# nygenome/Lancet2

Measured on AMD Instinct MI355X. Metric: microassembly windows/sec (whole node), higher is better.
Workload: dtype u8/i32 (f64 statistics)

## Files before the change

### lancet2_amd/csrc/assemble.hip

```cpp
#include <algorithm>
#include <cstdio>
#include <cstdlib>
#include <utility>
#include <vector>

#include "graph_ws.h"

namespace ma {

int run_build_pass(ma_ctx* ctx, const DBatch& b, GraphWs& ws, u32* counters_dev, int tc_log2_alloc);
int run_count_inst(ma_ctx* ctx, const DBatch& b, const GraphWs& ws, int win0, int nwin, u32* maxima_dev);
int run_select_active(ma_ctx* ctx, const GraphWs& ws, int win0, int nwin, const u32* gate_approx, u32* win_k,
                      u32* active, u32* n_active_dev);
int run_clean_pass(ma_ctx* ctx, const DBatch& b, const GraphWs& ws, const ma_asm_out_t& out);

namespace {

__global__ void k_init_out(ma_asm_out_t o, u32* win_flags, int n, u32 MC, u32 MH) {
  int const i = blockIdx.x * blockDim.x + threadIdx.x;
  if (i >= n) return;
  o.win_status[i] = MA_W_NO_HAPLOTYPE;
  o.win_k[i] = 0;
  o.win_ncomp[i] = 0;
  win_flags[i] = 0;
// ... 312 lines not shown

int launch_assemble(ma_ctx* ctx, const DBatch& b, const ma_asm_out_t& out, const u32* gate_approx) {
  int const n = b.n_windows;
  if (n == 0) return MA_OK;
  ma_params_t const& P = ctx->prm;
  int const S = P.num_samples;

  size_t const nseq = static_cast<size_t>(b.n_reads) + n;
  Carver cm{nullptr};
  auto carve_misc = [&](Carver& c, GraphWs& ws, u32** win_flags, u32** active, u32** counters) {
    ws.seq_inst_base = c.take<u32>(nseq + 1);
    ws.win_ninst = c.take<u32>(n);
    ws.win_nread_inst = c.take<u32>(n);
    *win_flags = c.take<u32>(n);
    *active = c.take<u32>(n);
    *counters = c.take<u32>(16);
    ws.rd_flag = c.take<u8>(static_cast<size_t>(b.n_reads) + 16);
  };
  GraphWs ws{};
  bool const nested = ctx->spec_k != nullptr;
  ws.win_kfirst = ctx->spec_k;
  u32 *win_flags = nullptr, *active = nullptr, *counters = nullptr;
  carve_misc(cm, ws, &win_flags, &active, &counters);
  MA_HIP(ctx, ctx->ws_nodes.reserve(cm.off + 4096));
  Carver cm2{static_cast<char*>(ctx->ws_nodes.p)};
  carve_misc(cm2, ws, &win_flags, &active, &counters);
  ws.win_flags = win_flags;
  ws.num_samples = S;

  hipLaunchKernelGGL(k_init_out, dim3((n + 63) / 64), dim3(64), 0, ctx->stream, out, win_flags, n, static_cast<u32>(P.max_comps),
                     static_cast<u32>(P.max_haps));
// ... 128 lines not shown
    size_t budget = stage_budget(0.60, ctx->ws_build.cap, size_t(48) << 30, ctx->hbm_share);
    if (const char* e = getenv("MA_WS_GB")) budget = static_cast<size_t>(atoi(e)) << 30;
    int chunk = static_cast<int>(std::max<size_t>(1, std::min<size_t>(n, budget / per_window)));
    MA_HIP(ctx, ctx->ws_build.reserve(per_window * static_cast<size_t>(chunk)));
    if (getenv("MA_VERBOSE"))
      fprintf(stderr, "[microasm] assemble: %d windows, %.2f MB/window, budget %.1f GB -> chunks of %d (nc %u, tc_log2 %d)\n", n,
              per_window / 1048576.0, budget / 1073741824.0, chunk, ws.nc, ws.tc_log2);

    for (int win0 = 0; win0 < n; win0 += chunk) {
      int const nwin = std::min(chunk, n - win0);
      ws.tc_log2 = tc_log2_alloc;
      ws.mc_log2 = mc_log2_alloc;
      Carver cw{static_cast<char*>(ctx->ws_build.p)};
      carve_ws(cw, ws, static_cast<size_t>(nwin));
      int const rungs = (P.max_k - P.min_k) / P.k_step + 1;
      for (int kpass = 0; kpass <= rungs; ++kpass) {
        MA_TRY_RC(run_select_active(ctx, ws, win0, nwin, gate_approx, out.win_k, active, counters + 8));
        u32 host_cnt[2] = {0, 0};
        MA_HIP(ctx, hipMemcpyAsync(host_cnt, counters + 8, 8, hipMemcpyDeviceToHost, ctx->stream));
        MA_HIP(ctx, ma_stream_sync(ctx));
        ws.n_active = static_cast<int>(host_cnt[0]);
        ws.active = active;
        if (host_cnt[1] == 0) break;
        if (!nested && kpass >= 1 && ws.n_active > 0 && static_cast<u32>(ws.n_active) <= kSpecPending && P.max_k > P.min_k &&
            !getenv("MA_NO_SPEC")) {
          u32 still = 0;
          MA_TRY_RC(speculate_tail(ctx, b, out, gate_approx, active, static_cast<u32>(ws.n_active), win_flags, counters + 8, &still));
          continue;
        }
        if (ws.n_active > 0) {
          if (!nested) ctx->stats[3] += static_cast<unsigned long long>(ws.n_active);
          if (nested || P.min_k != P.max_k) MA_TRY_RC(run_count_inst(ctx, b, ws, win0, nwin, counters));
          ws.tc_log2 = tc_log2_alloc;
          ws.mc_log2 = mc_log2_alloc;
          MA_TRY_RC(run_build_pass(ctx, b, ws, counters + 12, tc_log2_alloc));
          if (ctx->collect) {
            unsigned long long* acc = nullptr;
            MA_TRY_RC(ma_dev_stats(ctx, &acc));
            hipLaunchKernelGGL(k_workload_stats, dim3(ws.n_active), dim3(256), 0, ctx->stream, ws, acc);
          }
          MA_TRY_RC(run_clean_pass(ctx, b, ws, out));
        }
      }
    }
  }
  return MA_OK;
}

}
```

### lancet2_amd/csrc/build.hip

```cpp
#include "graph_ws.h"

namespace ma {

constexpr int kBT = 256;
__constant__ u64 c_phred_bits[256] = {
#include "../../include/ma_phred_lut.inc"
};

struct SeqInfo {
  u64 off;
  u32 len;
  u32 nk;
};

__device__ __forceinline__ u32 seq_count(const DBatch& b, int w) {
  return 1u + (b.read_win_off[w + 1] - b.read_win_off[w]);
}

__device__ __forceinline__ SeqInfo seq_info(const DBatch& b, int w, u32 s, int k) {
  SeqInfo si;
  if (s == 0) {
    si.off = b.ref_off[w];
    si.len = b.ref_off[w + 1] - b.ref_off[w];
  } else {
// ... 965 lines not shown
  i32* c_hint = reinterpret_cast<i32*>(c_ib + cache_cap);
  bool const cached = cache_cap != 0 && ns <= cache_cap;
  SeqInfo const rsi = seq_info(b, w, 0, k);
  for (u32 i = threadIdx.x; i < cnt_words; i += kSupT) l_cnt[i] = 0;
  for (u32 i = threadIdx.x; i < (kSupT / 64u) << ws.dd_log2; i += kSupT) l_dd[i] = 0;
  for (u32 i = threadIdx.x; i < xs_cap; i += kSupT) {
    l_xkey[i] = 0;
    l_xgrp[i] = 0;
  }
  if (threadIdx.x == 0) {
    xs_flag = ns > 65535u ? 1u : 0u;
    any_big = 0;
    gen_count = 0;
    genq_n = 0;
    edgeq_n = 0;
  }
  if (cached) {
    for (u32 sx = 1 + threadIdx.x; sx < ns; sx += kSupT) {
      u32 const r = b.read_win_off[w] + sx - 1;
      SeqInfo const si = seq_info(b, w, sx, k);
      c_meta[sx] = (b.read_flags[r] & 7u) | (ws.rd_flag[r] ? 8u : 0u) | (static_cast<u32>(b.read_sample[r]) << 8) | (min(si.nk, 0xFFFFu) << 16);
      c_qn[sx] = b.read_qname_id[r];
      c_ib[sx] = ws.seq_inst_base[base_idx + sx];
      c_hint[sx] = b.read_hint ? b.read_hint[r] : 0;
    }
  }
  __syncthreads();
  bool const hints = b.read_hint != nullptr && rsi.len <= ws.max_ref_len + 8;
  if (hints) {
    for (u32 s_idx = 1 + threadIdx.x; s_idx < ns; s_idx += kSupT) {
      u32 const r = b.read_win_off[w] + s_idx - 1;
      if (!(b.read_flags[r] & MA_RF_PASS)) continue;
      u32 const key = ((b.read_qname_id[r] << 1) | ((b.read_flags[r] & MA_RF_CASE) ? 1u : 0u)) + 1u;
      u32 h = (key * 2654435761u) >> xs_shift;
      bool done = false;
      for (u32 probe = 0; probe < xs_cap && !done; ++probe) {
        u32 cur = l_xkey[h];
        if (cur == 0) {
          u32 const old = atomicCAS(&l_xkey[h], 0u, key);
          if (old == 0) {
            l_xsmp[h] = b.read_sample[r];
            done = true;
            break;
          }
          cur = old;
        }
        if (cur == key) done = true; else h = (h + 1) & (xs_cap - 1);
      }
      if (!done) xs_flag = 1;
    }
  }
  __syncthreads();
  if (hints) {
    for (u32 s_idx = 1 + threadIdx.x; s_idx < ns; s_idx += kSupT) {
      u32 const r = b.read_win_off[w] + s_idx - 1;
      if (!(b.read_flags[r] & MA_RF_PASS)) continue;
      bool const leader = !(s_idx > 1 && same_group(b, r, r - 1));
      u32 const key = ((b.read_qname_id[r] << 1) | ((b.read_flags[r] & MA_RF_CASE) ? 1u : 0u)) + 1u;
      u32 h = (key * 2654435761u) >> xs_shift;
      for (u32 probe = 0; probe < xs_cap; ++probe) {
        u32 const cur = l_xkey[h];
        if (cur == key) {
          if (l_xsmp[h] != b.read_sample[r]) xs_flag = 1;
          if (leader && atomicAdd(&l_xgrp[h], 1u) != 0) xs_flag = 1;
          break;
        }
        if (cur == 0) break;
        h = (h + 1) & (xs_cap - 1);
      }
    }
  }
  if (hints && ns > kSeqCap) {
    for (u32 s_idx = 1 + kMmRunMax + threadIdx.x; s_idx < ns; s_idx += kSupT) {
      u32 const r = b.read_win_off[w] + s_idx - 1;
      u32 j = 0;
      while (j < kMmRunMax && same_group(b, r - j, r - j - 1)) ++j;
      if (j == kMmRunMax) xs_flag = 1;
    }
  }
  __syncthreads();
  bool const all_generic = !hints || xs_flag != 0;
  bool const qmode = !all_generic && !ws.mm_force_hbm && ns <= kSeqCap && tbl_log2(ws) <= 20;
  u32* const genq = ws.slowq + static_cast<size_t>(a) * ws.inst_stride;
  u32 const dd_cap = 1u << ws.dd_log2;
  uint2* const edgeq = reinterpret_cast<uint2*>(ws.slow_rec + static_cast<size_t>(a) * ws.inst_stride);

  u32* const l_leaders = l_mask;
  if (threadIdx.x == 0) n_leaders = 0;
  __syncthreads();
  for (u32 s_idx = 1 + threadIdx.x; s_idx < ns; s_idx += kSupT) {
    u32 const r0 = b.read_win_off[w] + s_idx - 1;
    if (!(b.read_flags[r0] & MA_RF_PASS)) continue;
    if (s_idx > 1 && same_group(b, r0, r0 - 1)) continue;
    l_leaders[atomicAdd(&n_leaders, 1u)] = s_idx;
    if (qmode) {
      u32 tot = 0;
      for (u32 j = 0; s_idx + j < ns && (j == 0 || same_group(b, r0, r0 + j)); ++j) tot += seq_info(b, w, s_idx + j, k).nk;
      if (tot > dd_cap / 4u * 3u) any_big = 1;
    }
  }
  __syncthreads();
  bool const qdedup = qmode && ws.graph_fused && !any_big && ws.win_nslots[a] <= kGrSlots;
  IPROF_T0();
  u32 const wave = threadIdx.x >> 6, lane = threadIdx.x & 63u;
  u32* const dd = l_dd + (wave << ws.dd_log2);
  u32 wave_gen = 0;
  auto same_group_c = [&](u32 sa, u32 sb) {
    u32 const ma_ = c_meta[sa], mb = c_meta[sb];
    return (mb & MA_RF_PASS) && c_qn[sa] == c_qn[sb] && ((ma_ ^ mb) & MA_RF_CASE) == 0 && ((ma_ ^ mb) & 0xFF00u) == 0;
  };
  for (u32 gi = wave; gi < n_leaders; gi += kSupT / 64) {
    u32 const s_idx = l_leaders[gi];
    u32 const r0 = b.read_win_off[w] + s_idx - 1;
    u32 gsize = 1;
    if (cached) {
      while (s_idx + gsize < ns && same_group_c(s_idx, s_idx + gsize)) gsize++;
    } else {
      while (s_idx + gsize < ns && same_group(b, r0, r0 + gsize)) gsize++;
    }
    bool generic = all_generic || gsize > 2;
    for (u32 gm = 0; gm < gsize && !generic; ++gm) {
      if (cached) {
        u32 const mt = c_meta[s_idx + gm];
        if ((mt & 8u) || (mt >> 16) > 32u * kMaskWords) generic = true;
      } else {
        SeqInfo const si = seq_info(b, w, s_idx + gm, k);
        if (ws.rd_flag[r0 + gm] || si.nk > 32u * kMaskWords) generic = true;
      }
    }
    u32 pre00 = 0, pre01 = 0, pre10 = 0, pre11 = 0;
    bool have_pre = cached && gsize <= 2;
    for (u32 gm = 0; gm < gsize && have_pre; ++gm) {
      u32 const nkc = c_meta[s_idx + gm] >> 16;
      if (nkc == 0xFFFFu || nkc > 128u) have_pre = false;
    }
    if (have_pre) {
      u32 const nka = c_meta[s_idx] >> 16, iba = c_ib[s_idx];
      pre00 = lane < nka ? inst_slot[iba + lane] : 0u;
      pre01 = 64u + lane < nka ? inst_slot[iba + 64u + lane] : 0u;
      if (gsize == 2) {
        u32 const nkb = c_meta[s_idx + 1] >> 16, ibb = c_ib[s_idx + 1];
        pre10 = lane < nkb ? inst_slot[ibb + lane] : 0u;
        pre11 = 64u + lane < nkb ? inst_slot[ibb + 64u + lane] : 0u;
      }
    }
    i32 hint0 = 0;
    u32 nk0 = 0;
    unsigned long long m0[kMaskWords / 2];
#pragma unroll
    for (int x = 0; x < kMaskWords / 2; ++x) m0[x] = 0;
    for (u32 gm = 0; gm < gsize; ++gm) {
      u32 const sx = s_idx + gm;
      u32 const r = r0 + gm;
      SeqInfo si;
      u32 ibase, smp, role;
      i32 hint_r;
      if (cached && (c_meta[sx] >> 16) != 0xFFFFu) {
        u32 const mt = c_meta[sx];
        si.nk = mt >> 16;
// ... 4 lines not shown
      } else {
        si = seq_info(b, w, sx, k);
        ibase = ws.seq_inst_base[base_idx + sx];
        smp = b.read_sample[r];
        role = (b.read_flags[r] & MA_RF_CASE) ? 1u : 0u;
        hint_r = hints ? b.read_hint[r] : 0;
      }
      if (si.nk == 0) continue;
      if (smp >= static_cast<u32>(S)) smp = S - 1;
      if (gm == 0) {
        hint0 = hints ? hint_r : 0;
        nk0 = si.nk;
      }
      for (u32 ob = 0; ob < si.nk; ob += 64) {
        u32 const o = ob + lane;
        u32 const word = have_pre ? (gm == 0 ? (ob == 0 ? pre00 : pre01) : (ob == 0 ? pre10 : pre11))
                                  : (o < si.nk ? inst_slot[ibase + o] : 0u);
        {
          u32 const dn = __shfl_down(word, 1, 64);
          u32 first_next;
          if (have_pre) first_next = ob == 0 ? __shfl(gm == 0 ? pre01 : pre11, 0, 64) : 0u;
          else first_next = ob + 64 < si.nk ? inst_slot[ibase + ob + 64] : 0u;
          u32 const nextw = lane == 63 ? first_next : dn;
          bool const pair = o + 1 < si.nk && !((word & kInstFast) && (nextw & kInstFast) &&
                                               (nextw & kInstSlotMask) == (word & kInstSlotMask) + 1u);
          unsigned long long const em = __ballot(pair);
          if (em) {
            u32 eb = 0;
            if (lane == 0) eb = atomicAdd(&edgeq_n, static_cast<u32>(__popcll(em)));
            eb = __shfl(eb, 0, 64);
            if (pair) edgeq[eb + static_cast<u32>(__popcll(em & ((1ull << lane) - 1ull)))] = edge_pack(ibase + o, word, nextw);
          }
        }
        bool const ef = (word & kInstErrFree) != 0;
        bool const to_gen = ef && (generic || !(word & kInstFast));
        u32 const p = word & kInstSlotMask;
        unsigned long long const gmask = __ballot(to_gen);
        if (qdedup) {
          if (gmask) {
            u32 const nslot = to_gen ? ((word & kInstFast) ? ref_slot_g[p] : p) : 0u;
            bool won = false;
            if (to_gen) {
              u32 const tag = gi + 1u, mine = (nslot << 11) | tag;
              u32 h = (nslot * 2654435761u) >> (32u - ws.dd_log2);
              for (;;) {
                u32 cur = dd[h];
// ... 3 lines not shown
                    won = true;
                    break;
                  }
                  cur = old;
                  if ((cur & 0x7FFu) != tag) continue;
                }
                if (cur == mine) break;
                h = (h + 1u) & (dd_cap - 1u);
              }
            }
            unsigned long long const wm = __ballot(won);
            if (wm) {
              u32 qb = 0;
              if (lane == 0) qb = atomicAdd(&genq_n, static_cast<u32>(__popcll(wm)));
              qb = __shfl(qb, 0, 64);
              if (won) genq[qb + static_cast<u32>(__popcll(wm & ((1ull << lane) - 1ull)))] = (nslot << 4) | (smp << 1) | role;
            }
          }
        } else if (qmode) {
          if (gmask) {
            u32 qb = 0;
            if (lane == 0) qb = atomicAdd(&genq_n, static_cast<u32>(__popcll(gmask)));
            qb = __shfl(qb, 0, 64);
            if (to_gen) {
              u32 const nslot = (word & kInstFast) ? ref_slot_g[p] : p;
              genq[qb + static_cast<u32>(__popcll(gmask & ((1ull << lane) - 1ull)))] = ((nslot << 11) | (s_idx - 1u)) + 1u;
            }
          }
        } else if (to_gen) {
          inst_slot[ibase + o] = word | kInstGen;
        }
        wave_gen += static_cast<u32>(__popcll(gmask));
        bool const fast = ef && !to_gen;
        bool dup = false;
        if (gm == 1 && nk0 > 0 && fast) {
          i64 const o0 = static_cast<i64>(p) - hint0;
          if (o0 >= 0 && o0 < static_cast<i64>(nk0)) {
            unsigned long long wd = 0;
#pragma unroll
            for (int x = 0; x < kMaskWords / 2; ++x) wd = (o0 >> 6) == x ? m0[x] : wd;
            dup = (wd >> (o0 & 63)) & 1ull;
// ... 8 lines not shown
        if (fast && !dup) {
          u32 const i1 = p * CW + smp, i2 = p * CW + S + role;
          atomicAdd(&l_cnt[i1 >> 1], 1u << ((i1 & 1u) * 16u));
          atomicAdd(&l_cnt[i2 >> 1], 1u << ((i2 & 1u) * 16u));
        }
      }
    }
  }
  if (lane == 0 && wave_gen) atomicAdd(&gen_count, wave_gen);
  IPROF_SYNC(27);
  if (threadIdx.x == 0) {
    bool const lds_ok = !all_generic && !ws.mm_force_hbm && (ns > kSeqCap || gen_count <= 4u * kMmLdsMax) && tbl_log2(ws) <= 20;
    ws.n_edgeq[a] = edgeq_n;
    ws.n_genq[a] = (qmode || qdedup) ? genq_n : 0u;
    ws.mm_mode[a] = qdedup ? (gen_count | 0x20000000u) : qmode ? (gen_count | 0x40000000u) : (gen_count | (lds_ok ? 0u : 0x80000000u));
    atomic_max_lazy(max_gen, gen_count);
    ws.mm_log2[a] = 0;
    if (!qmode && !lds_ok && gen_count) {
      atomic_max_lazy(max_gen + 1, gen_count);
      u32 lg = 10;
      while (lg < 31u && (1ull << lg) < static_cast<u64>(gen_count) * 4u / 3u + 16u) ++lg;
      unsigned long long const bytes = ((12ull << lg) + 255ull) & ~255ull;
      unsigned long long const at = atomicAdd(ws.mm_pool_used, bytes);
      if (at + bytes <= ws.mm_pool_bytes) {
        ws.mm_off[a] = at;
        ws.mm_log2[a] = lg;
      } else {
        atomicOr(&ws.win_flags[w], 4u);
      }
    }
// ... 823 lines not shown
__host__ __device__ inline u32 graph_lds_bytes(u32 inst_stride, u32 ref_stride, int S) {
  return 2u * kGrSlots + kGrSlots / 8u + ((2u * ref_stride + 15u) & ~15u) + graph_area_bytes(inst_stride, S) + 64u;
}
__global__ __launch_bounds__(kGrT) __attribute__((amdgpu_waves_per_eu(8, 8))) void k_graph(DBatch b, GraphWs ws, u32 min_node_cov) {
  extern __shared__ unsigned char lds_build[];
  __shared__ u32 sh[kGrT / 64];
  __shared__ u32 l_fail;
  int const a = blockIdx.x;
  int const w = static_cast<int>(ws.active[a]);
  int const S = ws.num_samples, CW = S + 2;
  int const tcl = tbl_log2(ws);
  u32 const tcap = ws.win_nslots[a];
  u32 const ninst = ws.win_ninst[w], nref = ninst - ws.win_nread_inst[w];
  u32 const nw = (ws.inst_stride + 31u) / 32u + 1u;
  if (threadIdx.x == 0) ws.gr_done[a] = 0;
  if ((ws.win_flags[w] & 4u) || tcap > kGrSlots || ninst > ws.inst_stride || ninst >= (1u << 22)) return;
  const u64* keys = ws.tbl_key + (static_cast<size_t>(a) << tcl);
  const u32* first = ws.tbl_first + (static_cast<size_t>(a) << tcl);
  u32* cnt = ws.tbl_cnt + (static_cast<size_t>(a) << tcl) * CW;
  const u32* inst_slot = ws.inst_slot + static_cast<size_t>(a) * ws.inst_stride;
  const u32* ref_slot_g = ws.ref_slot + static_cast<size_t>(a) * ws.ref_stride;
  size_t const nb = static_cast<size_t>(a) * ws.nc;
  u16* l_node = reinterpret_cast<u16*>(lds_build);
  u32* l_sign = reinterpret_cast<u32*>(lds_build + 2u * kGrSlots);
  u16* l_refn = reinterpret_cast<u16*>(lds_build + 2u * kGrSlots + kGrSlots / 8u);
  unsigned char* area = lds_build + 2u * kGrSlots + kGrSlots / 8u + ((2u * ws.ref_stride + 15u) & ~15u);
  u32* l_bits = reinterpret_cast<u32*>(area);
  u32* l_base = l_bits + nw;
  u16* l_pref = reinterpret_cast<u16*>(l_base + kSeqCap);
  u32* l_key = reinterpret_cast<u32*>(area);
  u32* l_ok = l_key + kGrSet;
// ... 89 lines not shown
      u32 const t = sh[x];
      if (x < wave) before += t;
      tot += t;
    }
    total_nodes = tot;
    u32 run = before + inc - mine;
    if (tot <= kGrSlots)
      for (u32 x = 0; x < per; ++x)
        if (w0 + x < nw) {
          l_pref[w0 + x] = static_cast<u16>(run);
          run += __popc(l_bits[w0 + x]);
        }
  }
  IPROF_SYNC(17);
  if (threadIdx.x == 0) ws.n_nodes[a] = total_nodes;
  if (total_nodes < ws.nc && total_nodes > kGrSlots) return;
  if (total_nodes >= ws.nc) {
    if (threadIdx.x == 0) {
      atomicOr(&ws.win_flags[w], 4u);
      ws.gr_done[a] = 1;
    }
    return;
  }
  u64 const win_read_off0 = b.read_off[b.read_win_off[w]];
#pragma unroll
  for (u32 j = 0; j < kPer; ++j) {
    if (!(surv & (1u << j))) continue;
    u32 const s = threadIdx.x + j * kGrT, ii = fi[j];
    u32 const idx = l_pref[ii >> 5] + __popc(l_bits[ii >> 5] & ((1u << (ii & 31u)) - 1u));
    l_node[s] = static_cast<u16>(idx);
    u32 const v = inst_slot[ii];
// ... 62 lines not shown
  for (u32 p = threadIdx.x; p + 1 < nref; p += kGrT) add_edge(p, edge_word(inst_slot[p]), edge_word(inst_slot[p + 1]));
  {
    const uint2* edgeq = reinterpret_cast<const uint2*>(ws.slow_rec + static_cast<size_t>(a) * ws.inst_stride);
    u32 const neq = ws.n_edgeq[a];
    constexpr int kU = 4;
    for (u32 q0 = threadIdx.x; q0 < neq; q0 += kGrT * kU) {
      uint2 e[kU];
#pragma unroll
      for (int u = 0; u < kU; ++u) e[u] = edgeq[min(q0 + u * kGrT, neq - 1u)];
#pragma unroll
      for (int u = 0; u < kU; ++u)
        if (q0 + u * kGrT < neq) add_edge(e[u].x & 0x3FFFFFu, (e[u].x >> 22) | ((e[u].y & 0x7FFu) << 10), e[u].y >> 11);
    }
  }
  IPROF_SYNC(20);
  if (l_fail) return;
  bool over = false;
  for (u32 i = threadIdx.x; i < kGrSet; i += kGrT) {
    u32 const key = l_key[i];
    if (key == kGrEmpty) continue;
    u32 const src = key >> 15, myok = l_ok[i];
    u32 r = 0, m = 0, h = h0_of(src);
    for (u32 probe = 0; probe < kGrSet; ++probe) {
      u32 const kk = l_key[h];
      if (kk == kGrEmpty) break;
      if ((kk >> 15) == src) {
        ++m;
        r += l_ok[h] < myok;
      }
      h = h + 1u == kGrSet ? 0u : h + 1u;
    }
    if (r < static_cast<u32>(kEdgeCap)) ws.nd_edge[(nb + src) * kEdgeCap + r] = key & 0x7FFFu;
    if (r == 0) ws.nd_nedge[nb + src] = static_cast<u8>(min(m, static_cast<u32>(kEdgeCap)));
    over |= m > static_cast<u32>(kEdgeCap);
  }
  if (over) atomicOr(&ws.win_flags[w], 4u);
  if (threadIdx.x == 0) ws.gr_done[a] = 1;
  IPROF(21);
}

int run_build_pass(ma_ctx* ctx, const DBatch& b, GraphWs& ws, u32* counters_dev, int tc_log2_alloc) {
  if (ws.n_active == 0) return MA_OK;
  int const S = ws.num_samples;
  size_t const A = ws.n_active;
  ws.tc_log2 = tc_log2_alloc;
  ws.max_slow = counters_dev;
  MA_HIP(ctx, hipMemsetAsync(counters_dev, 0, 12, ctx->stream));
  MA_HIP(ctx, hipMemsetAsync(ws.n_slow, 0, 4 * A, ctx->stream));
  MA_HIP(ctx, hipMemsetAsync(ws.mm_pool_used, 0, 8, ctx->stream));
  u32 const tiles_per_win = std::max<u32>(1, (ws.max_reads + 63) / 64);
  u32 const tile_cap = (64 * ws.max_read_len + 32 + 15) & ~15u;
  size_t const lds_c = ((ws.max_ref_len + 8 + 15) & ~15u) + 2048 + 2ull * tile_cap + 2 * 4ull * 64 * classify_mask_words(ws.max_read_len) + 64;
  if (lds_c > 160 * 1024) {
    ma_set_err(ctx, "ma_assemble_batch: reads too long for the LDS-staged classifier");
    return MA_ERR_PARAM;
  }
  if (lds_c > 65536)
    MA_HIP(ctx, hipFuncSetAttribute(reinterpret_cast<const void*>(k_classify), hipFuncAttributeMaxDynamicSharedMemorySize,
                                    static_cast<int>(lds_c)));
  ctx->tic("k_classify");
  hipLaunchKernelGGL(k_classify, dim3(ws.n_active * tiles_per_win), dim3(kClsT), lds_c, ctx->stream, b, ws, counters_dev,
                     tiles_per_win, tile_cap);
// ... 10 lines not shown
  while ((1u << xs_log2) < ws.max_reads + 2 && xs_log2 < 14) ++xs_log2;
  auto const sup_lds = [&](u32 lg) {
    return 2ull * ws.ref_stride * (S + 2) + 4 + (size_t(4 * (kSupT / 64)) << ws.dd_log2) + 4ull * (ws.max_reads + 2) + 9ull * (size_t(1) << lg) + 64 +
           16ull * sup_cache + 16;
  };
  while (xs_log2 > 10 && sup_lds(xs_log2) > 159u * 1024u) --xs_log2;
  size_t const lds_s = sup_lds(xs_log2);
  if (lds_s > 65536)
    MA_HIP(ctx, hipFuncSetAttribute(reinterpret_cast<const void*>(k_support), hipFuncAttributeMaxDynamicSharedMemorySize,
                                    static_cast<int>(lds_s)));
  ctx->tic("k_support");
  ws.mm_probe_max = getenv("MA_MM_PROBE_MAX") ? static_cast<u32>(std::max(1, atoi(getenv("MA_MM_PROBE_MAX")))) : kMmLdsCap;
  hipLaunchKernelGGL(k_support, dim3(ws.n_active), dim3(kSupT), lds_s, ctx->stream, b, ws, counters_dev + 1, sup_cache, xs_log2);
  ctx->toc();
  ctx->tic("k_mm_q");
  hipLaunchKernelGGL(k_mm_q<14>, dim3(std::min<u32>(static_cast<u32>(ws.n_active), 512u)), dim3(kMmT), 0, ctx->stream, b, ws);
  ctx->toc();
  if (ws.max_reads + 1u > kSeqCap) {
    ctx->tic("k_mm_lds");
    if (ws.mm_probe_max < kMmLdsCap) hipLaunchKernelGGL(k_mm_lds<true>, dim3(ws.n_active), dim3(kMmT), 0, ctx->stream, b, ws);
    else hipLaunchKernelGGL(k_mm_lds<false>, dim3(ws.n_active), dim3(kMmT), 0, ctx->stream, b, ws);
    ctx->toc();
  }
  ctx->tic("k_mm_hbm");
  hipLaunchKernelGGL(k_mm_hbm, dim3(ws.n_active), dim3(kBT), 0, ctx->stream, b, ws);
  ctx->toc();
  if (getenv("MA_VERBOSE")) {
    std::vector<u32> mm(A);
    u32 max_gen[2] = {0, 0};
    unsigned long long used = 0;
    MA_HIP(ctx, ma_stream_sync(ctx));
// ... 8 lines not shown
      tot += v & 0x1FFFFFFFu;
    }
    fprintf(stderr, "[ma] mate-mer sets: %zu windows, %zu need the HBM set (%zu by size), mean general instances %.0f, max %u / %u; pool %.1f of %.1f MB\n",
            A, nfb, big, static_cast<double>(tot) / static_cast<double>(A), max_gen[0], max_gen[1], used / 1048576.0, ws.mm_pool_bytes / 1048576.0);
  }
  MA_HIP(ctx, hipMemsetAsync(ws.gr_done, 0, 4 * A, ctx->stream));
  if (ws.graph_fused) {
    if (lds_g > 65536)
      MA_HIP(ctx, hipFuncSetAttribute(reinterpret_cast<const void*>(k_graph), hipFuncAttributeMaxDynamicSharedMemorySize,
                                      static_cast<int>(lds_g)));
    ctx->tic("k_graph");
    hipLaunchKernelGGL(k_graph, dim3(ws.n_active), dim3(kGrT), lds_g, ctx->stream, b, ws, static_cast<u32>(ctx->prm.min_node_cov));
    ctx->toc();
  }
  ctx->tic("k_graph_gen");
  hipLaunchKernelGGL(k_graph_gen, dim3(std::min<u32>(static_cast<u32>(ws.n_active), 512u)), dim3(kRankT), 0, ctx->stream, b, ws,
                     static_cast<u32>(ctx->prm.min_node_cov));
  ctx->toc();
  MA_HIP(ctx, hipGetLastError());
  return MA_OK;
}

int run_count_inst(ma_ctx* ctx, const DBatch& b, const GraphWs& ws, int win0, int nwin, u32* maxima_dev) {
  MA_HIP(ctx, hipMemsetAsync(maxima_dev, 0, 32, ctx->stream));
  hipLaunchKernelGGL(k_count_inst, dim3(nwin), dim3(kBT), 0, ctx->stream, b, ws, win0, nwin, maxima_dev);
  MA_HIP(ctx, hipGetLastError());
  return MA_OK;
}

int run_select_active(ma_ctx* ctx, const GraphWs& ws, int win0, int nwin, const u32* gate_approx, u32* win_k,
                      u32* active, u32* n_active_dev) {
// ... 9 lines not shown
```

### lancet2_amd/csrc/graph_ws.h

```cpp
#pragma once
#include "ma_internal.h"

namespace ma {

constexpr int kEdgeCap = 16;
constexpr u32 kNoNode = 0xFFFFFFFFu;
constexpr u32 kInstErrFree = 1u << 31;
constexpr u32 kInstPlus = 1u << 30;
constexpr u32 kInstFast = 1u << 29;
constexpr u32 kInstGen = 1u << 28;
constexpr u32 kInstLast = 1u << 27;
constexpr u32 kInstFirst = 1u << 26;
constexpr u32 kInstSlotMask = (1u << 26) - 1;
constexpr int kMaxSamples = 8;

struct GraphWs {
  int k;
  const u32* win_k;
  const u32* win_kfirst;
  u64 pk1;
  u64 pinv;
  int n_active;
  const u32* active;
  u32* seq_inst_base;
// ... 8 lines not shown
  u32 inst_stride;
  u64* tbl_key;
  u32* tbl_first;
  u32* tbl_cnt;
  u32* inst_slot;
  u32* slowq;
  u32* n_slow;
  u32* mm_mode;
  u32* win_nslots;
  uint4* slow_rec;
  u32 graph_fused;
  u32 dd_log2;
  u32* n_genq;
  u32* n_edgeq;
  u32* gr_done;
  u8* rd_flag;
  u8* mm_pool;
  unsigned long long mm_pool_bytes;
  unsigned long long* mm_pool_used;
  unsigned long long* mm_off;
  u32* mm_log2;
  u32 nc;
  u32* slot_node;
  u32* n_nodes;
  u32* nd_cnt;
  u32* nd_role;
  u32* nd_src;
  u8* nd_label;
  u8* nd_sign;
  u8* nd_nedge;
// ... 72 lines not shown
```

### lancet2_amd/csrc/ma_internal.h

```cpp
#pragma once
#include <hip/hip_runtime.h>
#include <cstdlib>

#include <cstdint>
#include <cstdio>
#include <mutex>
#include <string>
#include <vector>

#include "../../include/microasm.h"

namespace ma {

using u8 = uint8_t;
using u16 = uint16_t;
using u32 = uint32_t;
using u64 = uint64_t;
using i8 = int8_t;
using i16 = int16_t;
using i32 = int32_t;
using i64 = int64_t;
using f64 = double;
using f32 = float;

// ... 34 lines not shown
}

struct ma_ctx {
  ma_params_t prm;
  int device = 0;
  int memspace = MA_MEM_HOST;
  hipStream_t stream = nullptr;
  hipStream_t own_stream = nullptr;
  std::string err;
  std::mutex err_mu;
  ma::DevBuf in_stage[10];
  std::vector<ma::DevBuf> out_stage;
  ma::DevBuf ws_build, ws_nodes, ws_clean, ws_aln, ws_misc, ws_gen, ws_mm;
  ma::DevBuf spec_data, spec_out, spec_nodes;
  const uint32_t* spec_k = nullptr;
  ma::DevBuf ws_cx;
  double cx_gc = -1.0;
  int cx_ml = 0;
  std::vector<double> cx_host;
  std::vector<ma::KernelTimer> timers;
  size_t timers_used = 0;
  bool timing = true;
  bool accumulate = false;
  unsigned long long stats[8] = {0, 0, 0, 0, 0, 0, 0, 0};
  bool collect = false;
  ma::DevBuf dev_stats;
  bool dev_stats_clean = false;
  int n_lanes = 0;
  std::vector<ma_ctx*> lanes;
  ma::DevBuf lane_rwo;
// ... 137 lines not shown
```

Before: 290,400.

## Precompute group metadata in k_support leader pass and size fallback grids from last pass

In k_support, the leader scan now reads the LDS read cache. It computes group size, generic and precompute flags once per leader and packs them into the leader entry, which removes repeated global same_group walks. It also folds the hash-validation pass into that loop and adds a fully unrolled wave path for groups of up to two reads of 128 k-mers or fewer. Separately, device counters record how many windows actually took the k_mm_q and k_graph_gen fallback paths, and the next k-pass sizes those kernels' grids from that count. The goal is fewer idle blocks, at the cost of more counter traffic and a heuristic that could under-size a grid.

```diff
diff --git a/lancet2_amd/csrc/assemble.hip b/lancet2_amd/csrc/assemble.hip
--- a/lancet2_amd/csrc/assemble.hip
+++ b/lancet2_amd/csrc/assemble.hip
@@ -350,7 +350,7 @@
     ws.win_nread_inst = c.take<u32>(n);
     *win_flags = c.take<u32>(n);
     *active = c.take<u32>(n);
-    *counters = c.take<u32>(16);
+    *counters = c.take<u32>(24);
     ws.rd_flag = c.take<u8>(static_cast<size_t>(b.n_reads) + 16);
   };
   GraphWs ws{};
@@ -509,11 +509,16 @@
       Carver cw{static_cast<char*>(ctx->ws_build.p)};
       carve_ws(cw, ws, static_cast<size_t>(nwin));
       int const rungs = (P.max_k - P.min_k) / P.k_step + 1;
+      bool built = false;
       for (int kpass = 0; kpass <= rungs; ++kpass) {
         MA_TRY_RC(run_select_active(ctx, ws, win0, nwin, gate_approx, out.win_k, active, counters + 8));
-        u32 host_cnt[2] = {0, 0};
-        MA_HIP(ctx, hipMemcpyAsync(host_cnt, counters + 8, 8, hipMemcpyDeviceToHost, ctx->stream));
+        u32 host_cnt[9] = {0, 0, 0, 0, 0, 0, 0, 0, 0};
+        MA_HIP(ctx, hipMemcpyAsync(host_cnt, counters + 8, sizeof(host_cnt), hipMemcpyDeviceToHost, ctx->stream));
         MA_HIP(ctx, ma_stream_sync(ctx));
+        if (built) {
+          for (int x = 0; x < 2; ++x) ctx->route_last[x] = static_cast<int>(host_cnt[7 + x]);
+          built = false;
+        }
         ws.n_active = static_cast<int>(host_cnt[0]);
         ws.active = active;
         if (host_cnt[1] == 0) break;
@@ -529,6 +534,7 @@
           ws.tc_log2 = tc_log2_alloc;
           ws.mc_log2 = mc_log2_alloc;
           MA_TRY_RC(run_build_pass(ctx, b, ws, counters + 12, tc_log2_alloc));
+          built = true;
           if (ctx->collect) {
             unsigned long long* acc = nullptr;
             MA_TRY_RC(ma_dev_stats(ctx, &acc));
diff --git a/lancet2_amd/csrc/build.hip b/lancet2_amd/csrc/build.hip
--- a/lancet2_amd/csrc/build.hip
+++ b/lancet2_amd/csrc/build.hip
@@ -1003,7 +1003,9 @@
     gen_count = 0;
     genq_n = 0;
     edgeq_n = 0;
-  }
+    n_leaders = 0;
+  }
+  IPROF_T0();
   if (cached) {
     for (u32 sx = 1 + threadIdx.x; sx < ns; sx += kSupT) {
       u32 const r = b.read_win_off[w] + sx - 1;
@@ -1016,11 +1018,16 @@
   }
   __syncthreads();
   bool const hints = b.read_hint != nullptr && rsi.len <= ws.max_ref_len + 8;
+  auto same_group_c = [&](u32 sa, u32 sb) {
+    u32 const ma_ = c_meta[sa], mb = c_meta[sb];
+    return (mb & MA_RF_PASS) && c_qn[sa] == c_qn[sb] && ((ma_ ^ mb) & MA_RF_CASE) == 0 && ((ma_ ^ mb) & 0xFF00u) == 0;
+  };
   if (hints) {
     for (u32 s_idx = 1 + threadIdx.x; s_idx < ns; s_idx += kSupT) {
       u32 const r = b.read_win_off[w] + s_idx - 1;
-      if (!(b.read_flags[r] & MA_RF_PASS)) continue;
-      u32 const key = ((b.read_qname_id[r] << 1) | ((b.read_flags[r] & MA_RF_CASE) ? 1u : 0u)) + 1u;
+      u32 const fl = cached ? c_meta[s_idx] : static_cast<u32>(b.read_flags[r]);
+      if (!(fl & MA_RF_PASS)) continue;
+      u32 const key = (((cached ? c_qn[s_idx] : b.read_qname_id[r]) << 1) | ((fl & MA_RF_CASE) ? 1u : 0u)) + 1u;
       u32 h = (key * 2654435761u) >> xs_shift;
       bool done = false;
       for (u32 probe = 0; probe < xs_cap && !done; ++probe) {
@@ -1028,7 +1035,7 @@
         if (cur == 0) {
           u32 const old = atomicCAS(&l_xkey[h], 0u, key);
           if (old == 0) {
-            l_xsmp[h] = b.read_sample[r];
+            l_xsmp[h] = cached ? static_cast<u8>(fl >> 8) : b.read_sample[r];
             done = true;
             break;
           }
@@ -1040,98 +1047,257 @@
     }
   }
   __syncthreads();
-  if (hints) {
-    for (u32 s_idx = 1 + threadIdx.x; s_idx < ns; s_idx += kSupT) {
-      u32 const r = b.read_win_off[w] + s_idx - 1;
-      if (!(b.read_flags[r] & MA_RF_PASS)) continue;
-      bool const leader = !(s_idx > 1 && same_group(b, r, r - 1));
-      u32 const key = ((b.read_qname_id[r] << 1) | ((b.read_flags[r] & MA_RF_CASE) ? 1u : 0u)) + 1u;
-      u32 h = (key * 2654435761u) >> xs_shift;
-      for (u32 probe = 0; probe < xs_cap; ++probe) {
-        u32 const cur = l_xkey[h];
-        if (cur == key) {
-          if (l_xsmp[h] != b.read_sample[r]) xs_flag = 1;
-          if (leader && atomicAdd(&l_xgrp[h], 1u) != 0) xs_flag = 1;
-          break;
-        }
-        if (cur == 0) break;
-        h = (h + 1) & (xs_cap - 1);
-      }
-    }
-  }
-  if (hints && ns > kSeqCap) {
-    for (u32 s_idx = 1 + kMmRunMax + threadIdx.x; s_idx < ns; s_idx += kSupT) {
-      u32 const r = b.read_win_off[w] + s_idx - 1;
-      u32 j = 0;
-      while (j < kMmRunMax && same_group(b, r - j, r - j - 1)) ++j;
-      if (j == kMmRunMax) xs_flag = 1;
-    }
-  }
-  __syncthreads();
-  bool const all_generic = !hints || xs_flag != 0;
-  bool const qmode = !all_generic && !ws.mm_force_hbm && ns <= kSeqCap && tbl_log2(ws) <= 20;
+  auto const queue_mode = [&]() { return hints && xs_flag == 0 && !ws.mm_force_hbm && ns <= kSeqCap && tbl_log2(ws) <= 20; };
   u32* const genq = ws.slowq + static_cast<size_t>(a) * ws.inst_stride;
   u32 const dd_cap = 1u << ws.dd_log2;
   uint2* const edgeq = reinterpret_cast<uint2*>(ws.slow_rec + static_cast<size_t>(a) * ws.inst_stride);
 
   u32* const l_leaders = l_mask;
-  if (threadIdx.x == 0) n_leaders = 0;
-  __syncthreads();
-  for (u32 s_idx = 1 + threadIdx.x; s_idx < ns; s_idx += kSupT) {
-    u32 const r0 = b.read_win_off[w] + s_idx - 1;
-    if (!(b.read_flags[r0] & MA_RF_PASS)) continue;
-    if (s_idx > 1 && same_group(b, r0, r0 - 1)) continue;
-    l_leaders[atomicAdd(&n_leaders, 1u)] = s_idx;
-    if (qmode) {
-      u32 tot = 0;
-      for (u32 j = 0; s_idx + j < ns && (j == 0 || same_group(b, r0, r0 + j)); ++j) tot += seq_info(b, w, s_idx + j, k).nk;
+  if (cached) {
+    for (u32 s_idx = 1 + threadIdx.x; s_idx < ns; s_idx += kSupT) {
+      u32 const mt = c_meta[s_idx];
+      if (!(mt & MA_RF_PASS)) continue;
+      bool const leader = !(s_idx > 1 && same_group_c(s_idx, s_idx - 1));
+      if (hints) {
+        u32 const key = ((c_qn[s_idx] << 1) | ((mt & MA_RF_CASE) ? 1u : 0u)) + 1u;
+        u32 h = (key * 2654435761u) >> xs_shift;
+        for (u32 probe = 0; probe < xs_cap; ++probe) {
+          u32 const cur = l_xkey[h];
+          if (cur == key) {
+            if (l_xsmp[h] != static_cast<u8>(mt >> 8)) xs_flag = 1;
+            if (leader && atomicAdd(&l_xgrp[h], 1u) != 0) xs_flag = 1;
+            break;
+          }
+          if (cur == 0) break;
+          h = (h + 1) & (xs_cap - 1);
+        }
+      }
+      if (!leader) continue;
+      u32 gsize = 0, tot = 0;
+      bool gen = false, pre = true;
+      do {
+        u32 const mg = c_meta[s_idx + gsize];
+        u32 const nkc = mg >> 16;
+        tot += nkc;
+        gen |= (mg & 8u) || nkc > 32u * kMaskWords;
+        pre &= nkc <= 128u;
+        ++gsize;
+      } while (s_idx + gsize < ns && same_group_c(s_idx, s_idx + gsize));
+      gen |= gsize > 2;
+      pre &= gsize <= 2;
       if (tot > dd_cap / 4u * 3u) any_big = 1;
-    }
-  }
-  __syncthreads();
+      l_leaders[atomicAdd(&n_leaders, 1u)] = s_idx | (gsize << 12) | (gen ? 1u << 24 : 0u) | (pre ? 1u << 25 : 0u);
+    }
+  } else {
+    if (hints) {
+      for (u32 s_idx = 1 + threadIdx.x; s_idx < ns; s_idx += kSupT) {
+        u32 const r = b.read_win_off[w] + s_idx - 1;
+        if (!(b.read_flags[r] & MA_RF_PASS)) continue;
+        bool const leader = !(s_idx > 1 && same_group(b, r, r - 1));
+        u32 const key = ((b.read_qname_id[r] << 1) | ((b.read_flags[r] & MA_RF_CASE) ? 1u : 0u)) + 1u;
+        u32 h = (key * 2654435761u) >> xs_shift;
+        for (u32 probe = 0; probe < xs_cap; ++probe) {
+          u32 const cur = l_xkey[h];
+          if (cur == key) {
+            if (l_xsmp[h] != b.read_sample[r]) xs_flag = 1;
+            if (leader && atomicAdd(&l_xgrp[h], 1u) != 0) xs_flag = 1;
+            break;
+          }
+          if (cur == 0) break;
+          h = (h + 1) & (xs_cap - 1);
+        }
+      }
+    }
+    if (hints && ns > kSeqCap) {
+      for (u32 s_idx = 1 + kMmRunMax + threadIdx.x; s_idx < ns; s_idx += kSupT) {
+        u32 const r = b.read_win_off[w] + s_idx - 1;
+        u32 j = 0;
+        while (j < kMmRunMax && same_group(b, r - j, r - j - 1)) ++j;
+        if (j == kMmRunMax) xs_flag = 1;
+      }
+    }
+    __syncthreads();
+    bool const qmode_u = queue_mode();
+    for (u32 s_idx = 1 + threadIdx.x; s_idx < ns; s_idx += kSupT) {
+      u32 const r0 = b.read_win_off[w] + s_idx - 1;
+      if (!(b.read_flags[r0] & MA_RF_PASS)) continue;
+      if (s_idx > 1 && same_group(b, r0, r0 - 1)) continue;
+      l_leaders[atomicAdd(&n_leaders, 1u)] = s_idx;
+      if (qmode_u) {
+        u32 tot = 0;
+        for (u32 j = 0; s_idx + j < ns && (j == 0 || same_group(b, r0, r0 + j)); ++j) tot += seq_info(b, w, s_idx + j, k).nk;
+        if (tot > dd_cap / 4u * 3u) any_big = 1;
+      }
+    }
+  }
+  __syncthreads();
+  bool const qmode = queue_mode();
+  bool const all_generic = !hints || xs_flag != 0;
   bool const qdedup = qmode && ws.graph_fused && !any_big && ws.win_nslots[a] <= kGrSlots;
-  IPROF_T0();
+  IPROF(26);
   u32 const wave = threadIdx.x >> 6, lane = threadIdx.x & 63u;
+  unsigned long long const lane_lt = (1ull << lane) - 1ull;
   u32* const dd = l_dd + (wave << ws.dd_log2);
   u32 wave_gen = 0;
-  auto same_group_c = [&](u32 sa, u32 sb) {
-    u32 const ma_ = c_meta[sa], mb = c_meta[sb];
-    return (mb & MA_RF_PASS) && c_qn[sa] == c_qn[sb] && ((ma_ ^ mb) & MA_RF_CASE) == 0 && ((ma_ ^ mb) & 0xFF00u) == 0;
-  };
   for (u32 gi = wave; gi < n_leaders; gi += kSupT / 64) {
-    u32 const s_idx = l_leaders[gi];
+    u32 const lead = l_leaders[gi];
+    u32 const s_idx = cached ? (lead & 0xFFFu) : lead;
     u32 const r0 = b.read_win_off[w] + s_idx - 1;
     u32 gsize = 1;
+    bool generic, have_pre = false;
     if (cached) {
-      while (s_idx + gsize < ns && same_group_c(s_idx, s_idx + gsize)) gsize++;
+      gsize = (lead >> 12) & 0xFFFu;
+      generic = all_generic || ((lead >> 24) & 1u);
+      have_pre = (lead >> 25) & 1u;
     } else {
       while (s_idx + gsize < ns && same_group(b, r0, r0 + gsize)) gsize++;
-    }
-    bool generic = all_generic || gsize > 2;
-    for (u32 gm = 0; gm < gsize && !generic; ++gm) {
-      if (cached) {
-        u32 const mt = c_meta[s_idx + gm];
-        if ((mt & 8u) || (mt >> 16) > 32u * kMaskWords) generic = true;
-      } else {
+      generic = all_generic || gsize > 2;
+      for (u32 gm = 0; gm < gsize && !generic; ++gm) {
         SeqInfo const si = seq_info(b, w, s_idx + gm, k);
         if (ws.rd_flag[r0 + gm] || si.nk > 32u * kMaskWords) generic = true;
       }
     }
-    u32 pre00 = 0, pre01 = 0, pre10 = 0, pre11 = 0;
-    bool have_pre = cached && gsize <= 2;
-    for (u32 gm = 0; gm < gsize && have_pre; ++gm) {
-      u32 const nkc = c_meta[s_idx + gm] >> 16;
-      if (nkc == 0xFFFFu || nkc > 128u) have_pre = false;
-    }
     if (have_pre) {
-      u32 const nka = c_meta[s_idx] >> 16, iba = c_ib[s_idx];
-      pre00 = lane < nka ? inst_slot[iba + lane] : 0u;
-      pre01 = 64u + lane < nka ? inst_slot[iba + 64u + lane] : 0u;
-      if (gsize == 2) {
-        u32 const nkb = c_meta[s_idx + 1] >> 16, ibb = c_ib[s_idx + 1];
-        pre10 = lane < nkb ? inst_slot[ibb + lane] : 0u;
-        pre11 = 64u + lane < nkb ? inst_slot[ibb + 64u + lane] : 0u;
-      }
+      u32 const mta = c_meta[s_idx], mtb = c_meta[s_idx + 1];
+      u32 const iba = c_ib[s_idx], ibb = c_ib[s_idx + 1];
+      u32 const nka = mta >> 16, nkb = gsize == 2 ? mtb >> 16 : 0u;
+      i32 const hint0 = hints ? c_hint[s_idx] : 0;
+      u32 const smp = min((mta >> 8) & 0xFFu, static_cast<u32>(S) - 1u), role = (mta & MA_RF_CASE) ? 1u : 0u;
+      u32 word[4];
+      word[0] = lane < nka ? inst_slot[iba + lane] : 0u;
+      word[1] = 64u + lane < nka ? inst_slot[iba + 64u + lane] : 0u;
+      word[2] = lane < nkb ? inst_slot[ibb + lane] : 0u;
+      word[3] = 64u + lane < nkb ? inst_slot[ibb + 64u + lane] : 0u;
+      {
+        u32 nextw[4];
+        bool pair[4];
+        unsigned long long em[4];
+        u32 ne = 0;
+#pragma unroll
+        for (int j = 0; j < 4; ++j) {
+          u32 const nk = j < 2 ? nka : nkb, o = (j & 1) * 64u + lane;
+          u32 const dn = __shfl_down(word[j], 1, 64);
+          u32 const first_next = (j & 1) ? 0u : __shfl(word[j + 1], 0, 64);
+          nextw[j] = lane == 63 ? first_next : dn;
+          pair[j] = o + 1 < nk && !((word[j] & kInstFast) && (nextw[j] & kInstFast) &&
+                                    (nextw[j] & kInstSlotMask) == (word[j] & kInstSlotMask) + 1u);
+          em[j] = __ballot(pair[j]);
+          ne += static_cast<u32>(__popcll(em[j]));
+        }
+        if (ne) {
+          u32 eb = 0;
+          if (lane == 0) eb = atomicAdd(&edgeq_n, ne);
+          eb = __shfl(eb, 0, 64);
+#pragma unroll
+          for (int j = 0; j < 4; ++j) {
+            if (pair[j])
+              edgeq[eb + static_cast<u32>(__popcll(em[j] & lane_lt))] = edge_pack((j < 2 ? iba : ibb) + (j & 1) * 64u + lane, word[j], nextw[j]);
+            eb += static_cast<u32>(__popcll(em[j]));
+          }
+        }
+      }
+      bool to_gen[4], fast[4];
+      unsigned long long gmask[4];
+      u32 ng = 0;
+      bool via_ref = false;
+#pragma unroll
+      for (int j = 0; j < 4; ++j) {
+        bool const ef = (word[j] & kInstErrFree) != 0;
+        to_gen[j] = ef && (generic || !(word[j] & kInstFast));
+        fast[j] = ef && !to_gen[j];
+        via_ref |= to_gen[j] && (word[j] & kInstFast);
+        gmask[j] = __ballot(to_gen[j]);
+        ng += static_cast<u32>(__popcll(gmask[j]));
+      }
+      wave_gen += ng;
+      if (ng) {
+        u32 nslot[4];
+#pragma unroll
+        for (int j = 0; j < 4; ++j) nslot[j] = word[j] & kInstSlotMask;
+        if (__ballot(via_ref)) {
+          u32 rs[4];
+#pragma unroll
+          for (int j = 0; j < 4; ++j) rs[j] = ref_slot_g[(to_gen[j] && (word[j] & kInstFast)) ? nslot[j] : 0u];
+#pragma unroll
+          for (int j = 0; j < 4; ++j) nslot[j] = (to_gen[j] && (word[j] & kInstFast)) ? rs[j] : nslot[j];
+        }
+        if (qdedup) {
+          u32 const tag = gi + 1u;
+          u32 h[4], mine[4];
+          bool act[4], won[4];
+#pragma unroll
+          for (int j = 0; j < 4; ++j) {
+            mine[j] = (nslot[j] << 11) | tag;
+            h[j] = (nslot[j] * 2654435761u) >> (32u - ws.dd_log2);
+            act[j] = to_gen[j];
+            won[j] = false;
+          }
+          while (__ballot(act[0] || act[1] || act[2] || act[3])) {
+            u32 cur[4], old[4];
+#pragma unroll
+            for (int j = 0; j < 4; ++j) cur[j] = dd[h[j]];
+#pragma unroll
+            for (int j = 0; j < 4; ++j) old[j] = atomicCAS(&dd[h[j]], cur[j], (act[j] && (cur[j] & 0x7FFu) != tag) ? mine[j] : cur[j]);
+#pragma unroll
+            for (int j = 0; j < 4; ++j) {
+              bool const tried = act[j] && (cur[j] & 0x7FFu) != tag;
+              bool const got = tried && old[j] == cur[j];
+              u32 const eff = tried ? old[j] : cur[j];
+              bool const fin = got || eff == mine[j];
+              won[j] = won[j] || got;
+              if (act[j] && !fin && (eff & 0x7FFu) == tag) h[j] = (h[j] + 1u) & (dd_cap - 1u);
+              act[j] = act[j] && !fin;
+            }
+          }
+          unsigned long long wm[4];
+          u32 nw = 0;
+#pragma unroll
+          for (int j = 0; j < 4; ++j) {
+            wm[j] = __ballot(won[j]);
+            nw += static_cast<u32>(__popcll(wm[j]));
+          }
+          if (nw) {
+            u32 qb = 0;
+            if (lane == 0) qb = atomicAdd(&genq_n, nw);
+            qb = __shfl(qb, 0, 64);
+#pragma unroll
+            for (int j = 0; j < 4; ++j) {
+              if (won[j]) genq[qb + static_cast<u32>(__popcll(wm[j] & lane_lt))] = (nslot[j] << 4) | (smp << 1) | role;
+              qb += static_cast<u32>(__popcll(wm[j]));
+            }
+          }
+        } else if (qmode) {
+          u32 qb = 0;
+          if (lane == 0) qb = atomicAdd(&genq_n, ng);
+          qb = __shfl(qb, 0, 64);
+#pragma unroll
+          for (int j = 0; j < 4; ++j) {
+            if (to_gen[j]) genq[qb + static_cast<u32>(__popcll(gmask[j] & lane_lt))] = ((nslot[j] << 11) | (s_idx - 1u)) + 1u;
+            qb += static_cast<u32>(__popcll(gmask[j]));
+          }
+        } else {
+#pragma unroll
+          for (int j = 0; j < 4; ++j)
+            if (to_gen[j]) inst_slot[(j < 2 ? iba : ibb) + (j & 1) * 64u + lane] = word[j] | kInstGen;
+        }
+      }
+      unsigned long long const cm0 = __ballot(fast[0]), cm1 = __ballot(fast[1]);
+#pragma unroll
+      for (int j = 0; j < 4; ++j) {
+        u32 const p = word[j] & kInstSlotMask;
+        bool dup = false;
+        if (j >= 2) {
+          i64 const o0 = static_cast<i64>(p) - hint0;
+          unsigned long long const wd = (o0 >> 6) == 0 ? cm0 : cm1;
+          dup = o0 >= 0 && o0 < static_cast<i64>(nka) && ((wd >> (o0 & 63)) & 1ull);
+        }
+        if (fast[j] && !dup) {
+          u32 const i1 = p * CW + smp, i2 = p * CW + S + role;
+          atomicAdd(&l_cnt[i1 >> 1], 1u << ((i1 & 1u) * 16u));
+          atomicAdd(&l_cnt[i2 >> 1], 1u << ((i2 & 1u) * 16u));
+        }
+      }
+      continue;
     }
     i32 hint0 = 0;
     u32 nk0 = 0;
@@ -1166,13 +1332,10 @@
       }
       for (u32 ob = 0; ob < si.nk; ob += 64) {
         u32 const o = ob + lane;
-        u32 const word = have_pre ? (gm == 0 ? (ob == 0 ? pre00 : pre01) : (ob == 0 ? pre10 : pre11))
-                                  : (o < si.nk ? inst_slot[ibase + o] : 0u);
+        u32 const word = o < si.nk ? inst_slot[ibase + o] : 0u;
         {
           u32 const dn = __shfl_down(word, 1, 64);
-          u32 first_next;
-          if (have_pre) first_next = ob == 0 ? __shfl(gm == 0 ? pre01 : pre11, 0, 64) : 0u;
-          else first_next = ob + 64 < si.nk ? inst_slot[ibase + ob + 64] : 0u;
+          u32 const first_next = ob + 64 < si.nk ? inst_slot[ibase + ob + 64] : 0u;
           u32 const nextw = lane == 63 ? first_next : dn;
           bool const pair = o + 1 < si.nk && !((word & kInstFast) && (nextw & kInstFast) &&
                                                (nextw & kInstSlotMask) == (word & kInstSlotMask) + 1u);
@@ -1181,7 +1344,7 @@
             u32 eb = 0;
             if (lane == 0) eb = atomicAdd(&edgeq_n, static_cast<u32>(__popcll(em)));
             eb = __shfl(eb, 0, 64);
-            if (pair) edgeq[eb + static_cast<u32>(__popcll(em & ((1ull << lane) - 1ull)))] = edge_pack(ibase + o, word, nextw);
+            if (pair) edgeq[eb + static_cast<u32>(__popcll(em & lane_lt))] = edge_pack(ibase + o, word, nextw);
           }
         }
         bool const ef = (word & kInstErrFree) != 0;
@@ -1215,7 +1378,7 @@
               u32 qb = 0;
               if (lane == 0) qb = atomicAdd(&genq_n, static_cast<u32>(__popcll(wm)));
               qb = __shfl(qb, 0, 64);
-              if (won) genq[qb + static_cast<u32>(__popcll(wm & ((1ull << lane) - 1ull)))] = (nslot << 4) | (smp << 1) | role;
+              if (won) genq[qb + static_cast<u32>(__popcll(wm & lane_lt))] = (nslot << 4) | (smp << 1) | role;
             }
           }
         } else if (qmode) {
@@ -1225,7 +1388,7 @@
             qb = __shfl(qb, 0, 64);
             if (to_gen) {
               u32 const nslot = (word & kInstFast) ? ref_slot_g[p] : p;
-              genq[qb + static_cast<u32>(__popcll(gmask & ((1ull << lane) - 1ull)))] = ((nslot << 11) | (s_idx - 1u)) + 1u;
+              genq[qb + static_cast<u32>(__popcll(gmask & lane_lt))] = ((nslot << 11) | (s_idx - 1u)) + 1u;
             }
           }
         } else if (to_gen) {
@@ -1264,6 +1427,7 @@
     ws.n_edgeq[a] = edgeq_n;
     ws.n_genq[a] = (qmode || qdedup) ? genq_n : 0u;
     ws.mm_mode[a] = qdedup ? (gen_count | 0x20000000u) : qmode ? (gen_count | 0x40000000u) : (gen_count | (lds_ok ? 0u : 0x80000000u));
+    if (qmode && !qdedup && gen_count) atomicAdd(&ws.route_cnt[0], 1u);
     atomic_max_lazy(max_gen, gen_count);
     ws.mm_log2[a] = 0;
     if (!qmode && !lds_ok && gen_count) {
@@ -2117,7 +2281,10 @@
   u32 const ninst = ws.win_ninst[w], nref = ninst - ws.win_nread_inst[w];
   u32 const nw = (ws.inst_stride + 31u) / 32u + 1u;
   if (threadIdx.x == 0) ws.gr_done[a] = 0;
-  if ((ws.win_flags[w] & 4u) || tcap > kGrSlots || ninst > ws.inst_stride || ninst >= (1u << 22)) return;
+  if ((ws.win_flags[w] & 4u) || tcap > kGrSlots || ninst > ws.inst_stride || ninst >= (1u << 22)) {
+    if (threadIdx.x == 0) atomicAdd(&ws.route_cnt[1], 1u);
+    return;
+  }
   const u64* keys = ws.tbl_key + (static_cast<size_t>(a) << tcl);
   const u32* first = ws.tbl_first + (static_cast<size_t>(a) << tcl);
   u32* cnt = ws.tbl_cnt + (static_cast<size_t>(a) << tcl) * CW;
@@ -2237,7 +2404,10 @@
   }
   IPROF_SYNC(17);
   if (threadIdx.x == 0) ws.n_nodes[a] = total_nodes;
-  if (total_nodes < ws.nc && total_nodes > kGrSlots) return;
+  if (total_nodes < ws.nc && total_nodes > kGrSlots) {
+    if (threadIdx.x == 0) atomicAdd(&ws.route_cnt[1], 1u);
+    return;
+  }
   if (total_nodes >= ws.nc) {
     if (threadIdx.x == 0) {
       atomicOr(&ws.win_flags[w], 4u);
@@ -2330,7 +2500,10 @@
     }
   }
   IPROF_SYNC(20);
-  if (l_fail) return;
+  if (l_fail) {
+    if (threadIdx.x == 0) atomicAdd(&ws.route_cnt[1], 1u);
+    return;
+  }
   bool over = false;
   for (u32 i = threadIdx.x; i < kGrSet; i += kGrT) {
     u32 const key = l_key[i];
@@ -2361,7 +2534,12 @@
   size_t const A = ws.n_active;
   ws.tc_log2 = tc_log2_alloc;
   ws.max_slow = counters_dev;
-  MA_HIP(ctx, hipMemsetAsync(counters_dev, 0, 12, ctx->stream));
+  MA_HIP(ctx, hipMemsetAsync(counters_dev, 0, 20, ctx->stream));
+  ws.route_cnt = counters_dev + 3;
+  auto const route_grid = [&](int last) {
+    u32 const full = std::min<u32>(static_cast<u32>(ws.n_active), 512u);
+    return last < 0 ? full : std::min<u32>(full, std::max<u32>(16u, 2u * static_cast<u32>(last)));
+  };
   MA_HIP(ctx, hipMemsetAsync(ws.n_slow, 0, 4 * A, ctx->stream));
   MA_HIP(ctx, hipMemsetAsync(ws.mm_pool_used, 0, 8, ctx->stream));
   u32 const tiles_per_win = std::max<u32>(1, (ws.max_reads + 63) / 64);
@@ -2402,7 +2580,7 @@
   hipLaunchKernelGGL(k_support, dim3(ws.n_active), dim3(kSupT), lds_s, ctx->stream, b, ws, counters_dev + 1, sup_cache, xs_log2);
   ctx->toc();
   ctx->tic("k_mm_q");
-  hipLaunchKernelGGL(k_mm_q<14>, dim3(std::min<u32>(static_cast<u32>(ws.n_active), 512u)), dim3(kMmT), 0, ctx->stream, b, ws);
+  hipLaunchKernelGGL(k_mm_q<14>, dim3(route_grid(ctx->route_last[0])), dim3(kMmT), 0, ctx->stream, b, ws);
   ctx->toc();
   if (ws.max_reads + 1u > kSeqCap) {
     ctx->tic("k_mm_lds");
@@ -2441,7 +2619,7 @@
     ctx->toc();
   }
   ctx->tic("k_graph_gen");
-  hipLaunchKernelGGL(k_graph_gen, dim3(std::min<u32>(static_cast<u32>(ws.n_active), 512u)), dim3(kRankT), 0, ctx->stream, b, ws,
+  hipLaunchKernelGGL(k_graph_gen, dim3(route_grid(ws.graph_fused ? ctx->route_last[1] : -1)), dim3(kRankT), 0, ctx->stream, b, ws,
                      static_cast<u32>(ctx->prm.min_node_cov));
   ctx->toc();
   MA_HIP(ctx, hipGetLastError());
diff --git a/lancet2_amd/csrc/graph_ws.h b/lancet2_amd/csrc/graph_ws.h
--- a/lancet2_amd/csrc/graph_ws.h
+++ b/lancet2_amd/csrc/graph_ws.h
@@ -46,6 +46,7 @@
   u32* n_genq;
   u32* n_edgeq;
   u32* gr_done;
+  u32* route_cnt;
   u8* rd_flag;
   u8* mm_pool;
   unsigned long long mm_pool_bytes;
diff --git a/lancet2_amd/csrc/ma_internal.h b/lancet2_amd/csrc/ma_internal.h
--- a/lancet2_amd/csrc/ma_internal.h
+++ b/lancet2_amd/csrc/ma_internal.h
@@ -72,6 +72,7 @@
   ma::DevBuf ws_build, ws_nodes, ws_clean, ws_aln, ws_misc, ws_gen, ws_mm;
   ma::DevBuf spec_data, spec_out, spec_nodes;
   const uint32_t* spec_k = nullptr;
+  int route_last[2] = {-1, -1};
   ma::DevBuf ws_cx;
   double cx_gc = -1.0;
   int cx_ml = 0;
```

Result: no change. 293,200 (median of 6 runs) (+0.9%).
